# xbarin02/libdwt

Hardware: AMD Instinct MI355X
Metric: Gsamples/s (= % HBM3E BW) CDF 9/7 2-D fwd float, 8192^2 5-level (higher is better)
Workload: dtype f32

## Files before the change

### libdwt_amd/csrc/dwt_abi.hip

```cpp
#include "dwt_backend.h"

#include <climits>

using namespace dwtb;

namespace {
enum OptKind { kPlain, kSweep , kBool, kNonNegative };
struct Opt {
	const char *name;
	int *(*ref)(Ctx &);
	OptKind kind;
};
#define DWT_OPT(name_, member_, kind_) {name_, [](Ctx &c) -> int * { return &c.member_; }, kind_}
const Opt kOpts[] = {
	DWT_OPT("generic", force_generic, kSweep), DWT_OPT("eaw_two_pass", eaw_two_pass, kBool), DWT_OPT("feat_groups", feat_groups, kNonNegative), DWT_OPT("swt_fused", swt_fused, kBool), DWT_OPT("cond_fused", cond_fused, kPlain), DWT_OPT("timefreq_tiled", tf_tiled, kBool), DWT_OPT("cpt", tune.cpt, kSweep), DWT_OPT("tile_pairs", tune.tile_pairs, kSweep),
	DWT_OPT("waves", tune.waves, kSweep), DWT_OPT("xcd_swizzle", tune.xcd_swizzle, kSweep), DWT_OPT("ring", tune.ring, kSweep),
	DWT_OPT("ring_inv", tune.ring_inv, kSweep), DWT_OPT("inv_ll_temporal", tune.inv_ll_temporal, kSweep), DWT_OPT("inv_pairs", tune.inv_pairs, kSweep), DWT_OPT("nt", tune.nt, kSweep), DWT_OPT("nt_auto", tune.nt_auto, kSweep),
	DWT_OPT("fma", fma, kSweep), DWT_OPT("fused_d", fused_d, kPlain), DWT_OPT("ride_copy", ride_copy, kBool), DWT_OPT("ride_mib", ride_mib, kNonNegative), DWT_OPT("il_exact_borders", il_exact_borders, kPlain),
	DWT_OPT("il_inplace_shell", il_inplace_shell, kPlain), DWT_OPT("host_pipeline", host_pipeline, kPlain),
	DWT_OPT("tune_tiles", tune_tiles, kPlain), DWT_OPT("tune_in_call", tune_in_call, kBool), DWT_OPT("place_tries", place_tries, kPlain),
	DWT_OPT("place_min_mib", place_min_mib, kNonNegative), DWT_OPT("place_max_gib", place_max_gib, kNonNegative),
	DWT_OPT("vol_ip_waves", vol.ip_waves, kPlain), DWT_OPT("vol_tile_pairs", vol.tile_pairs, kPlain), DWT_OPT("vol_nt", vol.nt, kPlain),
	DWT_OPT("vol_fused", vol.fused, kPlain), DWT_OPT("vol_direct", vol.direct, kPlain), DWT_OPT("vol_whole", vol.whole, kPlain),
	DWT_OPT("vol_inplace_fused", vol.inplace_fused, kBool), DWT_OPT("vol_swizzle", vol.swizzle, kPlain), DWT_OPT("vol_rows", vol.rows, kPlain),
};
#undef DWT_OPT
const Opt *find_opt(const char *name)
{
	for (const Opt &o : kOpts)
		if (!strcmp(name, o.name))
			return &o;
	return nullptr;
}
}

#pragma GCC visibility push(default)
extern "C" {

const char *dwt_hip_last_error(void) { return g_err; }

int dwt_hip_device_count(void)
{
	int n = 0;
	if (hipGetDeviceCount(&n) != hipSuccess)
		return 0;
	return n;
}

int dwt_hip_init(void)
{
	if (g.inited)
// ... 445 lines not shown
```

### libdwt_amd/csrc/dwt_backend.h

```cpp
#pragma once
#include "../../include/libdwt_hip.h"
#include "dwt_kernels.h"

#include <hip/hip_runtime.h>
#include <stdarg.h>
#include <stdio.h>
#include <stdlib.h>
#include <string.h>
#include <algorithm>
#include <array>
#include <condition_variable>
#include <functional>
#include <initializer_list>
#include <map>
#include <mutex>
#include <thread>
#include <unistd.h>
#include <utility>
#include <vector>

namespace dwtb {
using namespace dwt;

struct Buf {
// ... 23 lines not shown
		return std::array{&stage_img, &ll[0], &ll[1], &frame_a, &frame_b, &vol_out, &vol_host[0], &vol_host[1], &eaw_w, &eaw_ll[0], &eaw_ll[1], &feat_ws, &swt_ws, &cond_ws, &band_ws};
	}
	hipEvent_t dl_ev[8] = {};
	hipEvent_t switch_ev = nullptr;
	hipStream_t up = nullptr, down = nullptr;
	hipEvent_t pipe_ev[3][16] = {};
	int host_pipeline = 1;
	void *pin = nullptr;
	size_t pin_bytes = 0;
	int feat_groups = 0;
	int tf_tiled = 1;
	int cond_fused = -1;
	int swt_fused = 1;
	SweepTuning tune;
	VolTuning vol;
	int force_generic = 0;
	int eaw_two_pass = 0;
	int fma = 0;
	int il_temporal = 0;
	int il_inplace_shell = 1;
	int il_exact_borders = 1;
	int tune_tiles = 1;
	std::map<unsigned long long, int> tile_cache;
	int place_tries = 4;
	int place_min_mib = 1024;
	int place_max_gib = 0;
	int tune_in_call = -1;
	bool tuning = false;
	bool placing = false;
	long stat_launches = 0, stat_allocs = 0;
	double place_ms[8] = {0};
	int place_n = 0, place_best = -1;
	int fused_d = 1;
	int ride_copy = 1;
	int ride_mib = 32;
	int prof_on = 0;
	std::vector<std::pair<hipEvent_t, hipEvent_t>> prof_events;
	std::vector<int> prof_tag;
	size_t prof_used = 0;
	double prof_ms = 0;
	int prof_launches = 0;
	double prof_level_ms[16] = {0};
	int prof_level_n[16] = {0};
};

extern thread_local Ctx g;
extern thread_local char g_err[512];
extern thread_local bool g_elems_are_32bit;

int fail(const char *fmt, ...);
int launched(hipError_t e, const char *family, const char *what);
int check_dev_align(std::initializer_list<const void *> ptrs, std::initializer_list<long> strides);
inline bool overlap(const void *a, size_t na, const void *b, size_t nb)
{
	const uintptr_t pa = (uintptr_t)a, pb = (uintptr_t)b;
	return na && nb && pa < pb + nb && pb < pa + na;
}

static inline bool wavelet_of(int id, Wavelet *w)
{
	if (id >= 0 && id <= 5) {
		*w = (Wavelet)id;
		return true;
	}
	if (id == DWT_HIP_INTERP53_S) {
		*w = kInterp53S;
// ... 34 lines not shown
	bool dense() const { return sox == six && soy == siy; }
};

int grow(Buf &b, size_t need);
void dev_free(void *p);
void drop(Buf &b);
int grant_range(const void *p, int owner, const int *devices, int n_devices);
int copy_rect_on(hipStream_t st, Img dst, long dx, long dy, Img src, long sx_, long sy_, long w, long h);
int copy_rect(Img dst, long dx, long dy, Img src, long sx_, long sy_, long w, long h);
int zero_rect(Img img, long x, long y, long w, long h);
struct Frame {
	void *p;
	long sx, sy;
	int es, w, h;
	bool dev;
};
int frame_check(const Frame &f);
int frame_pack(const Frame &f, void *dense, long pitch);
int frame_unpack(const Frame &f, const void *dense, long pitch);
inline long frame_pitch(long es, long w) { return align_up(es * w, 256); }
int frame_stage(const Frame &f, Buf &buf, Img *dense);
int frame_pack_stack(Frame f, int n, long plane_stride, void *stack, long pitch);
int frame_unpack_stack(Frame f, int n, long plane_stride, const void *stack, long pitch);
int host_volume_xfer(bool to_device, void *dev, size_t d_sy, size_t d_sz, void *host, size_t h_sy, size_t h_sz, int nx, int ny, int nz);
int generic_pass(Wavelet w, bool inverse, bool rows, Img in, Img out, int frame_w, int frame_h, int n_lines, int N, int hoff);
size_t ll_band_bytes(const Geom &ge, int k, int batch, int es);
int timed_forward(Wavelet w, Img s, Img d, const Geom &ge, int levels, int batch, long sb, long db, double *ms);
int place_ll_scratch(Wavelet w, Img s, Img d, const Geom &ge, int levels, int batch, long sb, long db);
int tune2d(Wavelet w, bool inverse, Img s, Img d, const Geom &ge, int levels, int batch, long sb, long db);
bool stream_is_capturing();
bool may_measure();
int tuned_tile_pairs(Wavelet w, const FwdLevelArgs &a);
int tuned_tile_pairs(Wavelet w, const InvLevelArgs &a);
void apply_tile_choice(int choice, SweepTuning *t, bool inverse);
int forward2d(Wavelet w, Img src, Img dst, const Geom &ge, int *jp, int decompose_one, int zero_padding, int batch, long src_bstride, long dst_bstride);
int inverse2d(Wavelet w, Img src, Img dst, const Geom &ge, int j_max, int decompose_one, int zero_padding, int batch, long src_bstride, long dst_bstride);
bool level_fused_ok(const Geom &ge, int j);
int transform1d(Wavelet w, bool inverse, const void *src, void *dst, long line_stride, long elem_stride, int n_lines,
	int so, int si, int *jp, int zero_padding);
int host_forward_pipelined(Wavelet w, const void *src, void *dst, int stride_x, int W, int H, int *jp, int decompose_one);
int host_inverse_pipelined(Wavelet w, const void *src, void *dst, int stride_x, int W, int H, int j_max, int decompose_one);
bool swt_fused_ok(const void *src, long ls, long es, int N);
int swt_device(Wavelet w, const char *src, long ls, long es, int n_lines, int N, int level0, int levels, char *dst_h, long h_es,
	char *dst_l, long l_es, int l_mode, long plane_stride, long dls);
int band_abs_median(const void *ptr, long bstride, int batch, long stride_x, int fw, int fh, int x0, int y0, int w, int h, float *med);
int prof_drain();
void prof_before(int level = 0);
void prof_after(int level = 0);
int check_inited();

}
```

### libdwt_amd/csrc/dwt_backend.hip

```cpp
#include "dwt_backend.h"

namespace dwtb {

thread_local Ctx g;
thread_local char g_err[512] = "";

int fail(const char *fmt, ...)
{
	va_list ap;
	va_start(ap, fmt);
	vsnprintf(g_err, sizeof(g_err), fmt, ap);
	va_end(ap);
	return 1;
}

int launched(hipError_t e, const char *family, const char *what)
{
	g.stat_launches++;
	return e == hipSuccess ? 0 : fail("%s %s launch failed: %s", family, what, hipGetErrorString(e));
}

int check_dev_align(std::initializer_list<const void *> ptrs, std::initializer_list<long> strides)
{
	bool ok = true;
// ... 171 lines not shown
	g.prof_used = 0;
	return 0;
}

long ll_pitch_elems(int w) { return align_up(w, 4); }
static char *ll_band(int k) { return (char *)g.ll[k].p; }

size_t ll_band_bytes(const Geom &ge, int k, int batch, int es)
{
	return (size_t)ll_pitch_elems(ge.Wo(k + 1)) * ge.Ho(k + 1) * es * batch + 64;
}

int ensure_ll(const Geom &ge, int batch, int es)
{
	for (int k = 0; k < 2; k++) {
		if (g.ll_external) {
			if (g.ll[k].bytes < ll_band_bytes(ge, k, batch, es))
				return fail("the caller's workspace (dwt_hip_set_workspace) is too small: band %d needs %zu bytes", k, ll_band_bytes(ge, k, batch, es));
			continue;
		}
		if (grow(g.ll[k], ll_band_bytes(ge, k, batch, es)))
			return 1;
	}
	return 0;
}

thread_local bool g_elems_are_32bit = true;

bool level_fused_ok(const Geom &ge, int j)
{
	return !g.force_generic && (g_elems_are_32bit || g.fused_d) && ge.Wi(j) == ge.Wo(j) && ge.Hi(j) == ge.Ho(j) && ge.Wo(j) >= 2 &&
		ge.Ho(j) >= 2;
}
int forward2d(Wavelet w, Img src, Img dst, const Geom &ge, int *jp, int decompose_one, int zero_padding,
	int batch, long src_bstride, long dst_bstride)
{
	const int so_min = ge.sox < ge.soy ? ge.sox : ge.soy, so_max = ge.sox > ge.soy ? ge.sox : ge.soy;
	const int j_limit = ceil_log2(decompose_one ? so_max : so_min);
	if (*jp < 0 || *jp > j_limit)
		*jp = j_limit;
	const int J = *jp;
	if (J == 0)
		return 0;
	const int es = elem_size(w);
	const bool dbl = es == 8;
	if (ensure_ll(ge, batch, es))
		return 1;

	int ll_in = -1;
	Img cur = src;
	RideCopy ride;
	auto carriers_from = [&](int j0) {
		int n = 0;
		for (int j = j0; j < J && level_fused_ok(ge, j); j++)
			n += !dbl && sweep_ride_ok(g.tune, ge.Wo(j), ge.Ho(j), batch, false);
		return n;
	};
	for (int j = 0; j < J; j++) {
		const int Wo = ge.Wo(j), Ho = ge.Ho(j), Wi = ge.Wi(j), Hi = ge.Hi(j);
		const int Wd = ge.Wo(j + 1), Hd = ge.Ho(j + 1);
		if (level_fused_ok(ge, j)) {
			const bool last = (j == J - 1) || !level_fused_ok(ge, j + 1);
			FwdLevelArgs a;
			a.W = Wo;
			a.H = Ho;
			a.batch = batch;
			bool detour = false;
			if (ll_in < 0) {
				a.in = cur.p;
				a.in_pitch = cur.sx / es;
				a.in_bstride = (cur.p == src.p ? src_bstride : dst_bstride) / es;
				detour = (cur.p == dst.p);
			} else {
				a.in = ll_band(ll_in);
				a.in_pitch = ll_pitch_elems(Wo);
				a.in_bstride = a.in_pitch * Ho;
			}
			Img hdst = dst;
			long h_bstride = dst_bstride;
			if (detour) {
				if (batch != 1)
					return fail("in-place batches are not supported; use distinct src and dst");
				if (grow(g.stage_img, (size_t)dst.sx * Ho))
					return 1;
				hdst = Img{(char *)g.stage_img.p, dst.sx, es};
				h_bstride = 0;
				a.temporal = (g.ride_copy && carriers_from(j + 1) > 0) ? 0 : 1;
			}
			a.out_h = hdst.p;
			a.h_pitch = hdst.sx / es;
			a.h_bstride = h_bstride / es;
			const int ll_out = last ? -1 : (ll_in < 0 ? (j & 1) : 1 - ll_in);
			if (last) {
				a.out_ll = hdst.p;
				a.ll_pitch = a.h_pitch;
				a.ll_bstride = a.h_bstride;
			} else {
				a.out_ll = ll_band(ll_out);
				a.ll_pitch = ll_pitch_elems(Wd);
				a.ll_bstride = a.ll_pitch * Hd;
			}
			SweepTuning tune = g.tune;
			if (!dbl && tune.tile_pairs <= 0)
				apply_tile_choice(tuned_tile_pairs(w, a), &tune, false);
			if (ride.on && ride.next < ride.total && !dbl && sweep_ride_ok(tune, Wo, Ho, batch, false)) {
				a.ride = &ride.r;
				a.ride_lo = ride.next;
				a.ride_hi = ride.next + ride.share((size_t)Wo * Ho * es, carriers_from(j + 1));
				ride.next = a.ride_hi;
			}
			prof_before(j);
			hipError_t e = dbl ? launch_fwd_level_d(w, a, tune, g.stream)
			                   : launch_fwd_level((g.fma && w == kCdf97S) ? kCdf97SFma : w, a, tune, g.stream);
			prof_after(j);
			if (e != hipSuccess)
				return fail("forward level %d launch failed: %s", j, hipGetErrorString(e));
			if (detour) {
				const Rect rc[3] = {{Wd, 0, Wd, 0, Wo - Wd, Ho}, {0, Hd, 0, Hd, Wd, Ho - Hd}, {0, 0, 0, 0, last ? Wd : 0, Hd}};
				ride.r = make_copy_rects(dst, hdst, rc, 3, 3);
				ride.total = copy_rects_plan(&ride.r);
				ride.next = 0;
				ride.on = g.ride_copy && ride.total > 0 && carriers_from(j + 1) > 0;
				if (!ride.on && copy_rects_on(g.stream, dst, hdst, rc, 3))
					return 1;
			}
			ll_in = ll_out;
			cur = dst;
			continue;
		}

		if (ride.flush())
			return 1;
		if (batch != 1)
			return fail("batched transforms need dense frames with both sides >= 2 at every level");
		if (ll_in >= 0) {
			Img s{ll_band(ll_in), ll_pitch_elems(Wo) * es, es};
			if (copy_rect(dst, 0, 0, s, 0, 0, Wo, Ho))
				return 1;
			ll_in = -1;
			cur = dst;
		}
		if (Wi == Wo && Hi == Ho && Wo >= 2 && Ho >= 2) {
			if (grow(g.stage_img, (size_t)dst.sx * Ho))
				return 1;
			const Img S{(char *)g.stage_img.p, dst.sx, dst.es};
			if (generic_pass(w, false, true, cur, S, Wo, Ho, Ho, Wi, Wd) || generic_pass(w, false, false, S, dst, Wo, Ho, Wo, Hi, Hd))
				return 1;
			cur = dst;
		} else {
			if (!skip_single(w) || Wo > 1) {
				if (generic_pass(w, false, true, cur, dst, Wo, Ho, Ho, Wi, Wd))
					return 1;
				cur = dst;
			}
			if (!skip_single(w) || Ho > 1) {
				if (generic_pass(w, false, false, cur, dst, Wo, Ho, Wo, Hi, Hd))
					return 1;
				cur = dst;
			}
		}
// ... 181 lines not shown
```

### libdwt_amd/csrc/dwt_kernels.h

```cpp
#pragma once
#include <hip/hip_runtime.h>
#include <stddef.h>

namespace dwt {

enum Wavelet { kCdf97S = 0, kCdf53I = 1, kCdf53S = 2, kCdf97D = 3, kCdf53D = 4, kCdf97I = 5,
	kCdf97SFma = 6 ,
	kCdf53SNew = 7 ,
	kCdf97IIp = 8 ,
	kInterp53S = 9  };

inline int elem_size(Wavelet w) { return (w == kCdf97D || w == kCdf53D) ? 8 : 4; }

struct SweepTuning {
	int cpt = 0;
	int tile_pairs = 0;
	int waves = 4;
	int xcd_swizzle = 1;
	int ring = 0;
	int nt = 7;
	int nt_auto = 1;
	int ring_inv = 8;
	int inv_pairs = 0;
	int inv_ll_temporal = 1;
// ... 31 lines not shown
	int il_ll = 0;
	int temporal = 0;
	int pair_lo = 0, pair_hi = 0;
	IlShell sh;
	const CopyRects *ride = nullptr;
	int ride_lo = 0, ride_hi = 0;
	int unused = 0;
	int out_step = 1;
};

struct InvLevelArgs {
	const void *in_ll;
	long ll_pitch, ll_bstride;
	const void *in_h;
	long h_pitch, h_bstride;
	void *out;
	long out_pitch, out_bstride;
	int W, H, batch;
	int interleaved = 0;
	int plain_ends = 0;
	int temporal_out = 0;
	int pair_lo = 0, pair_hi = 0;
	const CopyRects *ride = nullptr;
	int ride_lo = 0, ride_hi = 0;
	IlShell sh;
	int in_step = 1;
	const void *in_ll2 = nullptr;
	long ll2_pitch = 0;
};

struct IlStripArgs;
hipError_t launch_fwd_level(Wavelet w, const FwdLevelArgs &a, const SweepTuning &t, hipStream_t s, const IlStripArgs *strip = nullptr);

hipError_t launch_inv_level(Wavelet w, const InvLevelArgs &a, const SweepTuning &t, hipStream_t s, const IlStripArgs *strip = nullptr);
hipError_t launch_fwd_level_d(Wavelet w, const FwdLevelArgs &a, const SweepTuning &t, hipStream_t s);
hipError_t launch_inv_level_d(Wavelet w, const InvLevelArgs &a, const SweepTuning &t, hipStream_t s);
bool have_fused_inverse(Wavelet w);

hipError_t launch_line_pass(Wavelet w, bool inverse, const void *src, void *dst, long line_stride, long elem_stride,
	int n_lines, int N, int hoff, bool lanes_along_lines, hipStream_t s);

constexpr int N1D_MAX = 8192;
hipError_t launch_line_levels(Wavelet w, bool inverse, const void *src, void *dst, long line_stride, long elem_stride,
	int n_lines, int N, int levels, hipStream_t s);

hipError_t launch_eaw_line(bool inverse, const void *src, long ls, long es, int n_lines, int N, int hoff, float *tmp, float *w,
	bool lanes_along_lines, float alpha, hipStream_t s);
hipError_t launch_eaw_place(void *dst, long ls, long es, int n_lines, int N, int hoff, const float *tmp, bool lanes_along_lines, hipStream_t s);
struct EawLevelArgs {
	const float *in = nullptr;
	float *ll_out = nullptr, *det_out = nullptr, *wH_out = nullptr, *wV_out = nullptr;
	const float *ll = nullptr, *det = nullptr, *wH = nullptr, *wV = nullptr;
	float *out = nullptr;
	long pin = 0, pll = 0, pd = 0, pout = 0;
	long bi_in = 0, bi_ll = 0, bi_det = 0, bi_w = 0, bi_out = 0;
	int W = 0, H = 0, batch = 1;
};
hipError_t launch_eaw_level(bool inverse, const EawLevelArgs &a, float alpha, hipStream_t s);
hipError_t launch_eaw97_line(bool inverse, const void *src, long ls, long es, int n_lines, int N, int hoff, float *tmp, float *w,
	bool lanes_along_lines, float alpha, hipStream_t s);
hipError_t launch_eaw97_level(bool inverse, const EawLevelArgs &a, float alpha, hipStream_t s);

struct VolTuning {
	int cpt = 8;
	int tile_pairs = 0;
	int nt = -1;
// ... 241 lines not shown
```

### libdwt_amd/csrc/dwt_sweep2d.hip

```cpp
#include "dwt_sweep2d.h"

namespace dwt {

template <class W, bool INV>
__global__ __launch_bounds__(256) void k_line_pass(const char *__restrict__ src, char *__restrict__ dst,
	long line_stride, long elem_stride, int n_lines, int N, int hoff, int lanes_along_lines)
{
	using T = typename W::T;
	constexpr int K = W::K;
	const int fast = blockIdx.x * blockDim.x + threadIdx.x;
	const int slow = blockIdx.y;
	const int line = lanes_along_lines ? fast : slow;
	const int k = lanes_along_lines ? slow : fast;
	const int npairs = (N + 1) >> 1;
	if (line >= n_lines || k >= npairs)
		return;
	const char *s = src + (long)line * line_stride;
	char *d = dst + (long)line * line_stride;
	auto ld = [&](int idx) { return *(const T *)(s + (long)idx * elem_stride); };
	auto st = [&](int idx, T v) { *(T *)(d + (long)idx * elem_stride) = v; };
	const bool il = hoff < 0;

	if (N == 1) {
		if (W::kScaleSingle)
// ... 75 lines not shown
		if (v & 2)
			continue;
		constexpr int P = 2;
		const f2 ov = f2{row[0][v], row[0][v + P]}, ev = f2{row[1][v], row[1][v + P]};
		f2 s_[K], n_[K], lo2, hi2;
#pragma unroll
		for (int i = 0; i < K; i++)
			s_[i] = f2{st[i][v], st[i][v + P]};
		n_[0] = ev;
		n_[1] = ov + kk(0) * (tap(0, s_[0]) + ev);
		if constexpr (K == 4) {
			n_[2] = s_[0] + kk(1) * (tap(1, s_[1]) + n_[1]);
			n_[3] = s_[1] + kk(2) * (tap(2, s_[2]) + n_[2]);
			const f2 s2n = s_[2] + kk(3) * (tap(3, s_[3]) + n_[3]);
			lo2 = s2n * zl;
			hi2 = n_[3] * zh;
		} else {
			const f2 s1n = s_[0] + kk(1) * (tap(1, s_[1]) + n_[1]);
			lo2 = s1n * zl;
			hi2 = n_[1] * zh;
		}
#pragma unroll
		for (int i = 0; i < K; i++) {
			st[i][v] = n_[i][0];
			st[i][v + P] = n_[i][1];
		}
		lo[v] = lo2[0];
		lo[v + P] = lo2[1];
		hi[v] = hi2[0];
		hi[v + P] = hi2[1];
	}
}

template <class W, int CPT, int RING, int NT, bool IL, bool X>
static __device__ __forceinline__ void fwd_sweep_tile(const FwdLevelArgs &a, const SweepGeom &g)
{
	using T = typename W::T;
	constexpr int K = W::K;
	constexpr int kRing = RING;
	constexpr int kAhead = kRing / 2 - 1;
	constexpr int kLdAux = (NT & 2) ? 2 : 0;
	constexpr bool kNtStore = (NT & 1) != 0;
	[[maybe_unused]] constexpr bool kNtStoreLL = kNtStore && !(NT & 4);
	constexpr bool kShuffle = (NT & 8) != 0;
	constexpr int TW = 64 * CPT;
	constexpr int RS = TW + 8;
	constexpr int HK = (K + 1) & ~1;
	constexpr int NARR = CPT + 2 * HK;
	constexpr int kDmaPerIter = 2 * (CPT / 4 + 1);
	constexpr bool kPairRows = kIsSelEnds<W> && std::is_same<T, float>::value && has_coef_ends<W>::value && !std::is_base_of<Cdf97SFma, W>::value;
	extern __shared__ __attribute__((aligned(16))) char smem[];

	const int lane = threadIdx.x & 63, nwv = blockDim.x >> 6;
	const int wv = __builtin_amdgcn_readfirstlane(threadIdx.x >> 6);
	const int bid = tile_block_id(g.swz, X ? g.first : 0, g.tile_blocks);
	int tx, ty;
	if (g.wave_horiz) {
		const int ntxb = (g.ntx + nwv - 1) / nwv;
		tx = (bid % ntxb) * nwv + wv;
		ty = bid / ntxb;
	} else {
		tx = bid % g.ntx;
		ty = (bid / g.ntx) * nwv + wv;
	}
	const int img = blockIdx.y;
	const int Wd = (a.W + 1) >> 1, Hd = (a.H + 1) >> 1;
	const int A = ty * g.tile_pairs;
	if (A >= Hd || tx >= g.ntx)
		return;
	if (a.pair_hi > 0 && (A < a.pair_lo || A >= a.pair_hi))
		return;
	const int B = min(A + g.tile_pairs, Hd);
	const int c0 = tx * TW;
	const int n_iter = (B - A) + K;
	const int q0 = A - K / 2;

	const T *in = (const T *)a.in + (long)img * a.in_bstride;
	T *out_ll = (T *)a.out_ll + (long)img * a.ll_bstride;
	T *out_h = (T *)a.out_h + (long)img * a.h_bstride;

	char *ring = smem + (size_t)wv * kRing * RS * 4;
	const unsigned ring_off = lds_offset(ring);

	const int n_edge = min(4, c0 + TW - a.W);
	const int edge_col = kIsSelEnds<W> ? a.W - 2 - min(lane, 3) : reflect(a.W + min(lane, 3), a.W);
	const int halo_i = lane < 4 ? c0 - 4 + lane : c0 + TW + (lane & 3);
	const int halo_col = kIsSelEnds<W> ? reflect_near(halo_i, a.W) : reflect(halo_i, a.W);

	int islot = 0, rslot = 0;
	const bool tall = kIsSelEnds<W> || a.H >= 64;
	[[maybe_unused]] const bool shl = IL && a.sh.rows != nullptr;
	[[maybe_unused]] int halo_sh = -1;
	if (IL && shl)
		halo_sh = (halo_col >= c0 - 4 && halo_col < c0) ? 8 * (tx - 1) + (halo_col - (c0 - 4))
			: (halo_col >= c0 + TW && halo_col < c0 + TW + 4) ? 8 * tx + 4 + (halo_col - (c0 + TW)) : -1;
	auto issue = [&](int it) {
#pragma unroll
		for (int rr = 0; rr < 2; rr++) {
			const int ri = 2 * (q0 + it) - 1 + rr;
			const int r = tall ? reflect1(ri, a.H) : reflect(ri, a.H);
			char *lrow = ring + (size_t)(islot + rr) * RS * 4;
			const T *grow = in + (long)r * a.in_pitch;
			[[maybe_unused]] const T *hsrc = grow + halo_col;
			[[maybe_unused]] const T *rgt = nullptr;
			if (IL && shl) {
				if (r < 2 * A)
					grow = (const T *)a.sh.rows + (long)(9 * (ty - 1) + r - (2 * A - 5)) * a.sh.rows_pitch, hsrc = grow + halo_col;
				else if (r >= 2 * B)
					grow = (const T *)a.sh.rows + (long)(9 * ty + r - (2 * B - 5)) * a.sh.rows_pitch, hsrc = grow + halo_col;
				else if (r < kIlKeepTop)
					grow = (const T *)a.sh.top + (long)r * a.sh.top_pitch, hsrc = grow + halo_col;
				else {
					rgt = (const T *)a.sh.right + (long)r * a.sh.right_pitch - a.sh.right_x0;
					if (halo_sh >= 0)
						hsrc = (const T *)a.sh.cols + (long)r * a.sh.cols_pitch + halo_sh;
					else if (halo_col >= a.W - kIlKeepRight)
						hsrc = rgt + halo_col;
				}
			}
			[[maybe_unused]] const T *esrc = (IL && rgt) ? rgt + edge_col : grow + edge_col;
			const bool fix_right = IL && rgt && c0 + TW > a.W - kIlKeepRight;
			const row_rsrc_t rs = row_rsrc(grow, (unsigned)a.W * 4);
			if (kLdAux != 0 && it < K && A > 0) {
#pragma unroll
				for (int i = 0; i < CPT / 4; i++)
					dma16_row<0>(rs, (unsigned)(c0 + i * 256 + lane * 4) * 4, lrow + i * 1024);
				if (fix_right && lane < kIlKeepRight)
					dma4<0>(rgt + (a.W - kIlKeepRight + lane), lrow + (a.W - kIlKeepRight - c0) * 4);
				if (lane < n_edge)
					dma4<0>(esrc, lrow + (a.W - c0) * 4);
				if (lane < 8)
					dma4<0>(IL ? hsrc : grow + halo_col, lrow + TW * 4);
			} else {
#pragma unroll
				for (int i = 0; i < CPT / 4; i++)
					dma16_row<kLdAux>(rs, (unsigned)(c0 + i * 256 + lane * 4) * 4, lrow + i * 1024);
				if (fix_right && lane < kIlKeepRight)
					dma4<0>(rgt + (a.W - kIlKeepRight + lane), lrow + (a.W - kIlKeepRight - c0) * 4);
				if (lane < n_edge)
					dma4<kLdAux>(esrc, lrow + (a.W - c0) * 4);
				if (lane < 8)
					dma4<0>(IL ? hsrc : grow + halo_col, lrow + TW * 4);
			}
		}
		islot = islot + 2 >= kRing ? 0 : islot + 2;
	};

	T st[K][CPT];
#pragma unroll
	for (int s = 0; s < K; s++)
#pragma unroll
		for (int v = 0; v < CPT; v++)
			st[s][v] = 0;

	[[maybe_unused]] unsigned hends = 0;
	[[maybe_unused]] bool h_any = false, h_simple = false;
	constexpr unsigned kCand = (1u << HK) | (1u << (HK + CPT - 1));
	if constexpr (W::kEndForms) {
		hends = end_mask<NARR>(c0 + lane * CPT - HK, a.W);
		h_any = !a.plain_ends && __builtin_amdgcn_ballot_w64(hends != 0) != 0;
		h_simple = __builtin_amdgcn_ballot_w64((hends & ~(kCand | 1u | (1u << (NARR - 1)))) != 0) == 0;
	}
	[[maybe_unused]] bool e0 = false, e1 = false;
	[[maybe_unused]] T kh[K];
	if constexpr (kIsSelEnds<W>) {
		const unsigned m = end_mask_long<NARR>(c0 + lane * CPT - HK, a.W);
		e0 = (m >> HK) & 1;
		e1 = (m >> (HK + CPT - 1)) & 1;
		sel_coefs<W, false, HK>(kh, e0, e1);
	}
	[[maybe_unused]] auto row_is_end = [&](int r) {
		if (tall || kIsSelEnds<W>)
			return r == 0 || r == a.H - 1;
		const int rr = reflect(r, a.H);
		return rr == 0 || rr == a.H - 1;
	};

	for (int it = 0; it < kAhead && it < n_iter; it++)
		issue(it);

	for (int it = 0; it < n_iter; it++) {
		if (it + kAhead < n_iter) {
			issue(it + kAhead);
			DWT_WAIT_VMCNT(kAhead * kDmaPerIter);
		} else {
			DWT_WAIT_VMCNT(0);
		}

		T row[2][CPT];
		[[maybe_unused]] T xs[2][kPairRows ? NARR : 1];
#pragma unroll
		for (int rr = 0; rr < 2; rr++) {
			const unsigned base = ring_off + (unsigned)(rslot + rr) * RS * 4;
			const unsigned own = base + lane * CPT * 4;
			const unsigned la = lane == 0 ? base + TW * 4 : own - 16;
			const unsigned ra = lane == 63 ? base + TW * 4 + 16 : own + CPT * 4;
			T x[NARR];
			u4 L4, R4, O0, O1;
			if constexpr (kShuffle) {
				u4 H4;
				const unsigned ha = base + TW * 4 + (lane == 63 ? 16 : 0);
				if constexpr (CPT == 8) {
// ... 40 lines not shown
				if (__builtin_expect(!h_any, 1)) {
					lift_fwd_regs<W, NARR>(x, 0u);
				} else if (h_simple) {
					DWT_END_PATH();
					lift_fwd_regs<W, NARR, kCand>(x, hends);
				} else {
					DWT_END_PATH();
					lift_fwd_regs<W, NARR>(x, hends);
				}
			} else if constexpr (kIsSelEnds<W>) {
				lift_regs_sel<W, NARR, false, HK, HK + CPT - 1>(x, e0, e1, kh);
			} else {
				lift_fwd_regs<W, NARR>(x, 0u);
			}
#pragma unroll
			for (int v = 0; v < CPT; v++)
				row[rr][v] = W::fwd_scale(v & 1, x[HK + v]);
		}

		if constexpr (kPairRows) {
			typedef float f2 __attribute__((ext_vector_type(2)));
			f2 x2[NARR];
#pragma unroll
			for (int j = 0; j < NARR; j++)
				x2[j] = f2{xs[0][j], xs[1][j]};
#pragma unroll
			for (int s_ = 0; s_ < K; s_++) {
#pragma unroll
				for (int j = s_ + 1; j <= NARR - 2 - s_; j += 2) {
					if (j == HK)
						x2[j] = x2[j] + kh[s_] * ((e0 ? f2{-0.0f, -0.0f} : x2[j - 1]) + x2[j + 1]);
					else if (j == HK + CPT - 1)
						x2[j] = x2[j] + kh[s_] * (x2[j - 1] + (e1 ? f2{-0.0f, -0.0f} : x2[j + 1]));
					else
						x2[j] = x2[j] + W::fk(s_) * (x2[j - 1] + x2[j + 1]);
				}
			}
			const float ze = W::fwd_scale(0, 1.0f), zo = W::fwd_scale(1, 1.0f);
#pragma unroll
			for (int v = 0; v < CPT; v++) {
				const f2 sc = x2[HK + v] * ((v & 1) ? zo : ze);
				row[0][v] = sc[0];
				row[1][v] = sc[1];
			}
		}
		rslot = rslot + 2 >= kRing ? 0 : rslot + 2;

		[[maybe_unused]] bool vend[K] = {};
		[[maybe_unused]] bool v_any = false;
		if constexpr (W::kEndForms) {
#pragma unroll
			for (int s_ = 0; s_ < K; s_++) {
				vend[s_] = row_is_end(2 * (q0 + it) - 1 - s_);
				v_any = !a.plain_ends && (v_any || vend[s_]);
			}
		}
		T lo[CPT], hi[CPT];
		auto vertical = [&](auto ends_tag) {
			constexpr bool ENDS = decltype(ends_tag)::value;
			if constexpr (kPairRows && !ENDS && K != 1) {
				vertical_pairs<W, CPT>(row, st, lo, hi);
				return;
			}
#pragma unroll
			for (int v = 0; v < CPT; v++) {
				const T ov = row[0][v], ev = row[1][v];
// ... 109 lines not shown
#pragma unroll
					for (int e = 0; e < CPT; e += 4)
						store8_row<false>(dl, (unsigned)(c0 + lane * CPT) * 2 + e * 2, u2{to_bits(lo[e]), to_bits(lo[e + 2])});
				}
			} else
			if (it >= K && (!X || A + it - K >= kIlKeepTop / 2)) {
				const int k = A + it - K;
				const unsigned cb = (unsigned)(c0 + lane * CPT) * 4;
				const T *r0 = out_h + (long)(2 * k) * a.h_pitch;
				const unsigned row_bytes = (unsigned)(X ? a.W - kIlKeepRight : a.W) * 4;
				const row_rsrc_t d0 = row_rsrc(r0, row_bytes);
#pragma unroll
				for (int e = 0; e < CPT; e += 4) {
					const u4 v4{to_bits(lo[e]), to_bits(lo[e + 1]), to_bits(lo[e + 2]), to_bits(lo[e + 3])};
					if (a.il_ll == 2)
						store16_row<false>(d0, cb + e * 4, v4);
					else
						store16_row<kNtStore>(d0, cb + e * 4, v4);
				}
				if (2 * k + 1 < a.H) {
					const row_rsrc_t d1 = row_rsrc(r0 + a.h_pitch, row_bytes);
#pragma unroll
					for (int e = 0; e < CPT; e += 4)
						store16_row<kNtStore>(d1, cb + e * 4, u4{to_bits(hi[e]), to_bits(hi[e + 1]), to_bits(hi[e + 2]), to_bits(hi[e + 3])});
				}
				if (a.il_ll) {
					const row_rsrc_t dl = row_rsrc(out_ll + (long)k * a.ll_pitch, (unsigned)(X ? (a.W - kIlKeepRight + 1) >> 1 : Wd) * 4);
#pragma unroll
					for (int e = 0; e < CPT; e += 4)
						store8_row<false>(dl, cb / 2 + e * 2, u2{to_bits(lo[e]), to_bits(lo[e + 2])});
				}
			}
		} else
		if (it >= K) {
			const int k = A + it - K;
			const unsigned clb = (unsigned)((c0 + lane * CPT) >> 1) * 4;
			const T *top = out_h + (long)k * a.h_pitch, *bot = out_h + (long)(Hd + k) * a.h_pitch;
			const unsigned nlb = (unsigned)Wd * 4, nhb = (unsigned)(a.W >> 1) * 4;
			const row_rsrc_t dll = row_rsrc(out_ll + (long)k * a.ll_pitch, nlb), dhl = row_rsrc(top + Wd, nhb);
			const bool hrow = k < (a.H >> 1);
			if constexpr (CPT == 8) {
				store16_row<kNtStoreLL>(dll, clb, u4{to_bits(lo[0]), to_bits(lo[2]), to_bits(lo[4]), to_bits(lo[6])});
				store16_row<kNtStore>(dhl, clb, u4{to_bits(lo[1]), to_bits(lo[3]), to_bits(lo[5]), to_bits(lo[7])});
				if (hrow) {
					store16_row<kNtStore>(row_rsrc(bot, nlb), clb, u4{to_bits(hi[0]), to_bits(hi[2]), to_bits(hi[4]), to_bits(hi[6])});
					store16_row<kNtStore>(row_rsrc(bot + Wd, nhb), clb, u4{to_bits(hi[1]), to_bits(hi[3]), to_bits(hi[5]), to_bits(hi[7])});
				}
			} else {
				store8_row<kNtStoreLL>(dll, clb, u2{to_bits(lo[0]), to_bits(lo[2])});
				store8_row<kNtStore>(dhl, clb, u2{to_bits(lo[1]), to_bits(lo[3])});
				if (hrow) {
					store8_row<kNtStore>(row_rsrc(bot, nlb), clb, u2{to_bits(hi[0]), to_bits(hi[2])});
					store8_row<kNtStore>(row_rsrc(bot + Wd, nhb), clb, u2{to_bits(hi[1]), to_bits(hi[3])});
				}
			}
		}
	}
}

template <class W, int CPT, int RING, int NT, bool IL, bool X>
static __device__ __forceinline__ void fwd_sweep_any_tile(const FwdLevelArgs &a, const SweepGeom &g)
{
	if constexpr (W::kEndForms) {
		if (a.plain_ends)
			fwd_sweep_tile<PlainEnds<W>, CPT, RING, NT, IL, X>(a, g);
		else if (a.W % CPT == 0 && a.W >= 64 && a.H >= 64)
			fwd_sweep_tile<SelEnds<W>, CPT, RING, NT, IL, X>(a, g);
		else
			fwd_sweep_tile<W, CPT, RING, NT, IL, X>(a, g);
	} else
		fwd_sweep_tile<W, CPT, RING, NT, IL, X>(a, g);
}

template <class W, int CPT, int RING, int NT, bool IL = false>
__global__ __launch_bounds__(256) void k_fwd_sweep(FwdLevelArgs a, SweepGeom g)
{
	fwd_sweep_any_tile<W, CPT, RING, NT, IL, false>(a, g);
}

template <class W, int CPT, int RING, int NT>
__global__ __launch_bounds__(256) void k_fwd_sweep_r(FwdLevelArgs a, SweepGeom g, CopyRects r)
{
	if ((int)blockIdx.x >= g.tile_blocks) {
		ride_copy_block(r, (int)blockIdx.x - g.tile_blocks);
		return;
	}
	fwd_sweep_any_tile<W, CPT, RING, NT, false, false>(a, g);
}

template <class W, int CPT, int RING, int NT>
__global__ __launch_bounds__(256) void k_fwd_sweep_x(FwdLevelArgs a, SweepGeom g, IlStripArgs strip)
{
	if ((int)blockIdx.x < g.first) {
		il_strip_wave<W, false>(strip, blockIdx.x * (blockDim.x >> 6) + (threadIdx.x >> 6));
		return;
	}
	fwd_sweep_any_tile<W, CPT, RING, NT, true, true>(a, g);
}

template <class W, int CPT, int RING, int NT, bool IL = false>
static hipError_t fwd_launch(const FwdLevelArgs &a, const SweepGeom &g, dim3 grid, int waves, hipStream_t s)
{
	const size_t lds = (size_t)waves * RING * (64 * CPT + 8) * 4;
	if constexpr (!IL && RING == 8 && (NT == 7 || NT == 3)) {
		if (a.ride && a.ride_hi > a.ride_lo) {
			if (hipError_t e = allow_lds((const void *)k_fwd_sweep_r<W, CPT, RING, NT>, lds))
				return e;
			SweepGeom gr = g;
			gr.tile_blocks = (int)grid.x;
			CopyRects r = *a.ride;
// ... 65 lines not shown
	if (g.wave_horiz)
		grid = dim3(((g.ntx + waves - 1) / waves) * nty, a.batch);
	else
		grid = dim3(g.ntx * ((nty + waves - 1) / waves), a.batch);
	if (a.sh.rows && (!a.interleaved || a.batch != 1 || a.out_step != 1 || g.tile_pairs != a.sh.tile_pairs))
		return hipErrorInvalidValue;
	if (a.ride && a.ride_hi > a.ride_lo && (a.interleaved || a.batch != 1 || waves != 4 || tt.ring != 8 || a.temporal || (tt.nt & 8)))
		return hipErrorInvalidValue;
	if (a.interleaved) {
		if constexpr (std::is_same<W, Cdf97S>::value || std::is_same<W, Cdf53SNew>::value) {
			if (strip) {
				if (a.batch != 1 || a.W < 64 || a.H < 64)
					return hipErrorInvalidValue;
				return tt.ring == 16 ? fwd_launch_x<W, 16>(a, g, grid, waves, *strip, s) : fwd_launch_x<W, 8>(a, g, grid, waves, *strip, s);
			}
		}
		if (strip)
			return hipErrorInvalidValue;
		if constexpr (std::is_base_of<Cdf97S, W>::value || std::is_base_of<Cdf53S, W>::value) {
			if (tt.ring == 16)
				return fwd_launch<W, 4, 16, 3, true>(a, g, grid, waves, s);
			return fwd_launch<W, 4, 8, 3, true>(a, g, grid, waves, s);
		} else {
			return hipErrorInvalidValue;
		}
	}
	if (strip)
		return hipErrorInvalidValue;
	if (tt.nt_auto && (tt.nt & 12) == 4 && (size_t)a.batch * ((a.W + 1) / 2) * ((a.H + 1) / 2) * sizeof(typename W::T) >= ((size_t)1 << 30))
		tt.nt = 3;
	return cpt == 8 ? fwd_pick<W, 8>(a, g, grid, waves, tt, s) : fwd_pick<W, 4>(a, g, grid, waves, tt, s);
}

bool sweep_ride_ok(const SweepTuning &t, int W, int H, int batch, bool inverse)
{
	if (batch != 1 || W < 2 || H < 2 || !(t.waves >= 1 && t.waves <= 4 ? t.waves == 4 : true) || (t.nt & 8))
		return false;
	if (inverse)
		return t.ring_inv != 16;
	if (t.ring == 16)
		return false;
	if (t.ring == 8)
		return true;
	const int cpt = pick_cpt(t, W, false);
	const int tp = pick_tile_pairs(t, W, H, cpt, 1);
	const long ntx = (W + 64 * cpt - 1) / (64 * cpt), nty = ((H + 1) / 2 + tp - 1) / tp;
	return !(ntx >= 4 && ntx * nty >= 3072);
}

int il_sweep_tile_pairs(const SweepTuning &t, int W, int H, bool inverse)
{
	return pick_tile_pairs(t, W, H, 4, 1, inverse, true);
}

hipError_t launch_fwd_level(Wavelet w, const FwdLevelArgs &a, const SweepTuning &t, hipStream_t s, const IlStripArgs *strip)
{
	if (strip && w != kCdf97S && w != kCdf53SNew)
		return hipErrorInvalidValue;
	switch (w) {
	case kCdf97S: return fwd_level_t<Cdf97S>(a, t, s, strip);
	case kCdf53I: return fwd_level_t<Cdf53I>(a, t, s);
	case kCdf53S: return fwd_level_t<Cdf53S>(a, t, s);
	case kCdf97I: return fwd_level_t<Cdf97I>(a, t, s);
	case kCdf97SFma: return fwd_level_t<Cdf97SFma>(a, t, s);
	case kCdf53SNew: return a.interleaved ? fwd_level_t<Cdf53SNew>(a, t, s, strip) : hipErrorInvalidValue;
	case kInterp53S: return a.interleaved ? hipErrorInvalidValue : fwd_level_t<Interp53S>(a, t, s);
// ... 7 lines not shown
```

### libdwt_amd/csrc/dwt_tuning.hip

```cpp
#include "dwt_backend.h"

namespace dwtb {

bool may_measure()
{
	if (g.tune_in_call < 0) {
		const char *e = getenv("DWT_HIP_TUNE");
		g.tune_in_call = (e && atoi(e) > 0) ? 1 : 0;
	}
	return g.tuning || g.tune_in_call > 0;
}

struct TileCand {
	int pairs, cpt, ring;
};
static int pack_choice(const TileCand &c) { return c.pairs | (c.cpt << 16) | (c.ring << 24); }

void apply_tile_choice(int choice, SweepTuning *t, bool inverse)
{
	if (choice <= 0)
		return;
	t->tile_pairs = choice & 0xffff;
	if ((choice >> 16) & 0xff)
		t->cpt = (choice >> 16) & 0xff;
// ... 42 lines not shown
			fprintf(stderr, "tune %s W %d: %d pairs, cpt %d, ring %d: %.1f us%s\n", inverse ? "inv" : "fwd", (int)((key >> 38) & 0xfffff), c.pairs, c.cpt, c.ring,
				ms * 1e3, ok ? "" : " (failed)");
		if (ok && (!best || ms < best_ms)) {
			best = pack_choice(c);
			best_ms = ms;
		}
	}
	hipEventDestroy(e0);
	hipEventDestroy(e1);
	(void)hipGetLastError();
	g.tile_cache[key] = best;
	return best;
}

static unsigned long long tile_key(Wavelet w, bool inverse, int W, int H, int batch)
{
	return ((unsigned long long)w << 59) ^ ((unsigned long long)inverse << 58) ^ ((unsigned long long)W << 38) ^ ((unsigned long long)H << 18) ^ (unsigned long long)batch;
}

static bool tunable(int W, int H, int batch, int interleaved)
{
	return g.tune_tiles && !interleaved && (size_t)W * H * batch * sizeof(float) >= ((size_t)512 << 20) && W >= 1024 && H >= 256;
}

int tuned_tile_pairs(Wavelet w, const FwdLevelArgs &a)
{
	if (!tunable(a.W, a.H, a.batch, a.interleaved))
		return 0;
	const Wavelet wk = (g.fma && w == kCdf97S) ? kCdf97SFma : w;
	return tune_tile_pairs(tile_key(w, false, a.W, a.H, a.batch), false, {{64, 0, 0}, {32, 0, 0}, {16, 0, 0}},
		[&](const SweepTuning &t) { return launch_fwd_level(wk, a, t, g.stream); });
}

int tuned_tile_pairs(Wavelet w, const InvLevelArgs &a)
{
	if (!tunable(a.W, a.H, a.batch, a.interleaved))
		return 0;
	const Wavelet wk = (g.fma && w == kCdf97S) ? kCdf97SFma : w;
	return tune_tile_pairs(tile_key(w, true, a.W, a.H, a.batch), true, {{16, 0, 0}, {32, 0, 0}, {8, 0, 0}, {16, 8, 0}, {32, 8, 0}},
		[&](const SweepTuning &t) { return launch_inv_level(wk, a, t, g.stream); });
}
int timed_forward(Wavelet w, Img s, Img d, const Geom &ge, int levels, int batch, long sb, long db, double *ms)
{
	hipEvent_t e0, e1;
	HIP_TRY(hipEventCreate(&e0));
	HIP_TRY(hipEventCreate(&e1));
	int rc = 0;
	g.placing = true;
	for (int r = 0; r < 2 && !rc; r++) {
		int j = levels;
		hipEventRecord(e0, g.stream);
		rc = forward2d(w, s, d, ge, &j, 0, 0, batch, sb, db);
		hipEventRecord(e1, g.stream);
	}
	g.placing = false;
	float t = 0;
	if (!rc && (hipEventSynchronize(e1) != hipSuccess || hipEventElapsedTime(&t, e0, e1) != hipSuccess))
		rc = fail("timing a placement trial failed: %s", hipGetErrorString(hipGetLastError()));
	hipEventDestroy(e0);
	hipEventDestroy(e1);
	*ms = t;
	return rc;
}

static size_t place_jump(int k)
{
// ... 140 lines not shown
```

Before: 575.8.

## Fuse first two forward CDF 9/7 levels into one sweep kernel

Adds a fused kernel that computes level 0 of the float CDF 9/7 forward transform and feeds its LL rows straight into a level-1 lifting pass held in registers. Level 1's horizontal lift uses cross-lane shuffles and its vertical lift a register ring, writing both levels' detail bands and the level-1 LL. This avoids the HBM write and re-read of the level-0 LL band and one kernel launch, at the cost of overlapping tiles with halo recomputation, warm-up rows and higher register pressure. A heuristic gate and a separate tile-size tuning entry decide when the fused pair is used.

```diff
diff --git a/libdwt_amd/csrc/dwt_abi.hip b/libdwt_amd/csrc/dwt_abi.hip
--- a/libdwt_amd/csrc/dwt_abi.hip
+++ b/libdwt_amd/csrc/dwt_abi.hip
@@ -16,7 +16,7 @@
 	DWT_OPT("generic", force_generic, kSweep), DWT_OPT("eaw_two_pass", eaw_two_pass, kBool), DWT_OPT("feat_groups", feat_groups, kNonNegative), DWT_OPT("swt_fused", swt_fused, kBool), DWT_OPT("cond_fused", cond_fused, kPlain), DWT_OPT("timefreq_tiled", tf_tiled, kBool), DWT_OPT("cpt", tune.cpt, kSweep), DWT_OPT("tile_pairs", tune.tile_pairs, kSweep),
 	DWT_OPT("waves", tune.waves, kSweep), DWT_OPT("xcd_swizzle", tune.xcd_swizzle, kSweep), DWT_OPT("ring", tune.ring, kSweep),
 	DWT_OPT("ring_inv", tune.ring_inv, kSweep), DWT_OPT("inv_ll_temporal", tune.inv_ll_temporal, kSweep), DWT_OPT("inv_pairs", tune.inv_pairs, kSweep), DWT_OPT("nt", tune.nt, kSweep), DWT_OPT("nt_auto", tune.nt_auto, kSweep),
-	DWT_OPT("fma", fma, kSweep), DWT_OPT("fused_d", fused_d, kPlain), DWT_OPT("ride_copy", ride_copy, kBool), DWT_OPT("ride_mib", ride_mib, kNonNegative), DWT_OPT("il_exact_borders", il_exact_borders, kPlain),
+	DWT_OPT("fma", fma, kSweep), DWT_OPT("fused_d", fused_d, kPlain), DWT_OPT("fuse01", fuse01, kPlain), DWT_OPT("ride_copy", ride_copy, kBool), DWT_OPT("ride_mib", ride_mib, kNonNegative), DWT_OPT("il_exact_borders", il_exact_borders, kPlain),
 	DWT_OPT("il_inplace_shell", il_inplace_shell, kPlain), DWT_OPT("host_pipeline", host_pipeline, kPlain),
 	DWT_OPT("tune_tiles", tune_tiles, kPlain), DWT_OPT("tune_in_call", tune_in_call, kBool), DWT_OPT("place_tries", place_tries, kPlain),
 	DWT_OPT("place_min_mib", place_min_mib, kNonNegative), DWT_OPT("place_max_gib", place_max_gib, kNonNegative),
diff --git a/libdwt_amd/csrc/dwt_backend.h b/libdwt_amd/csrc/dwt_backend.h
--- a/libdwt_amd/csrc/dwt_backend.h
+++ b/libdwt_amd/csrc/dwt_backend.h
@@ -79,6 +79,7 @@
 	double place_ms[8] = {0};
 	int place_n = 0, place_best = -1;
 	int fused_d = 1;
+	int fuse01 = 1;
 	int ride_copy = 1;
 	int ride_mib = 32;
 	int prof_on = 0;
@@ -179,6 +180,7 @@
 bool may_measure();
 int tuned_tile_pairs(Wavelet w, const FwdLevelArgs &a);
 int tuned_tile_pairs(Wavelet w, const InvLevelArgs &a);
+int tuned_tile_pairs01(Wavelet w, const FwdLevelArgs &a);
 void apply_tile_choice(int choice, SweepTuning *t, bool inverse);
 int forward2d(Wavelet w, Img src, Img dst, const Geom &ge, int *jp, int decompose_one, int zero_padding, int batch, long src_bstride, long dst_bstride);
 int inverse2d(Wavelet w, Img src, Img dst, const Geom &ge, int j_max, int decompose_one, int zero_padding, int batch, long src_bstride, long dst_bstride);
diff --git a/libdwt_amd/csrc/dwt_backend.hip b/libdwt_amd/csrc/dwt_backend.hip
--- a/libdwt_amd/csrc/dwt_backend.hip
+++ b/libdwt_amd/csrc/dwt_backend.hip
@@ -227,6 +227,20 @@
 	return !g.force_generic && (g_elems_are_32bit || g.fused_d) && ge.Wi(j) == ge.Wo(j) && ge.Hi(j) == ge.Ho(j) && ge.Wo(j) >= 2 &&
 		ge.Ho(j) >= 2;
 }
+static bool pair01_ok(Wavelet w, const Geom &ge, int J, int batch)
+{
+	const int W = ge.Wo(0), H = ge.Ho(0);
+	if (!g.fuse01 || g.fma || J < 2 || !level_fused_ok(ge, 0) || !level_fused_ok(ge, 1) || !fwd01_can(w, W, H))
+		return false;
+	const SweepTuning &t = g.tune;
+	if (t.cpt == 4 || t.ring == 8 || (t.nt & 8) || (t.tile_pairs & 1))
+		return false;
+	if (g.fuse01 >= 2)
+		return true;
+	const long ntx = (W + 511) / 512, nty = ((H >> 1) + 63) / 64;
+	return fwd01_tiles(W) * 10 <= ntx * 11 && ntx * nty * batch >= 32768;
+}
+
 int forward2d(Wavelet w, Img src, Img dst, const Geom &ge, int *jp, int decompose_one, int zero_padding,
 	int batch, long src_bstride, long dst_bstride)
 {
@@ -255,7 +269,9 @@
 		const int Wo = ge.Wo(j), Ho = ge.Ho(j), Wi = ge.Wi(j), Hi = ge.Hi(j);
 		const int Wd = ge.Wo(j + 1), Hd = ge.Ho(j + 1);
 		if (level_fused_ok(ge, j)) {
-			const bool last = (j == J - 1) || !level_fused_ok(ge, j + 1);
+			const bool pair = j == 0 && ll_in < 0 && cur.p != dst.p && pair01_ok(w, ge, J, batch);
+			const int jl = pair ? j + 1 : j;
+			const bool last = (jl == J - 1) || !level_fused_ok(ge, jl + 1);
 			FwdLevelArgs a;
 			a.W = Wo;
 			a.H = Ho;
@@ -285,19 +301,19 @@
 			a.out_h = hdst.p;
 			a.h_pitch = hdst.sx / es;
 			a.h_bstride = h_bstride / es;
-			const int ll_out = last ? -1 : (ll_in < 0 ? (j & 1) : 1 - ll_in);
+			const int ll_out = last ? -1 : (ll_in < 0 ? (jl & 1) : 1 - ll_in);
 			if (last) {
 				a.out_ll = hdst.p;
 				a.ll_pitch = a.h_pitch;
 				a.ll_bstride = a.h_bstride;
 			} else {
 				a.out_ll = ll_band(ll_out);
-				a.ll_pitch = ll_pitch_elems(Wd);
-				a.ll_bstride = a.ll_pitch * Hd;
+				a.ll_pitch = ll_pitch_elems(ge.Wo(jl + 1));
+				a.ll_bstride = a.ll_pitch * ge.Ho(jl + 1);
 			}
 			SweepTuning tune = g.tune;
 			if (!dbl && tune.tile_pairs <= 0)
-				apply_tile_choice(tuned_tile_pairs(w, a), &tune, false);
+				apply_tile_choice(pair ? tuned_tile_pairs01(w, a) : tuned_tile_pairs(w, a), &tune, false);
 			if (ride.on && ride.next < ride.total && !dbl && sweep_ride_ok(tune, Wo, Ho, batch, false)) {
 				a.ride = &ride.r;
 				a.ride_lo = ride.next;
@@ -305,8 +321,9 @@
 				ride.next = a.ride_hi;
 			}
 			prof_before(j);
-			hipError_t e = dbl ? launch_fwd_level_d(w, a, tune, g.stream)
-			                   : launch_fwd_level((g.fma && w == kCdf97S) ? kCdf97SFma : w, a, tune, g.stream);
+			hipError_t e = pair ? launch_fwd01(a, tune, g.stream)
+			             : dbl  ? launch_fwd_level_d(w, a, tune, g.stream)
+			                    : launch_fwd_level((g.fma && w == kCdf97S) ? kCdf97SFma : w, a, tune, g.stream);
 			prof_after(j);
 			if (e != hipSuccess)
 				return fail("forward level %d launch failed: %s", j, hipGetErrorString(e));
@@ -321,6 +338,7 @@
 			}
 			ll_in = ll_out;
 			cur = dst;
+			j = jl;
 			continue;
 		}
 
diff --git a/libdwt_amd/csrc/dwt_kernels.h b/libdwt_amd/csrc/dwt_kernels.h
--- a/libdwt_amd/csrc/dwt_kernels.h
+++ b/libdwt_amd/csrc/dwt_kernels.h
@@ -87,6 +87,10 @@
 struct IlStripArgs;
 hipError_t launch_fwd_level(Wavelet w, const FwdLevelArgs &a, const SweepTuning &t, hipStream_t s, const IlStripArgs *strip = nullptr);
 
+bool fwd01_can(Wavelet w, int W, int H);
+int fwd01_tiles(int W);
+hipError_t launch_fwd01(const FwdLevelArgs &a, const SweepTuning &t, hipStream_t s);
+
 hipError_t launch_inv_level(Wavelet w, const InvLevelArgs &a, const SweepTuning &t, hipStream_t s, const IlStripArgs *strip = nullptr);
 hipError_t launch_fwd_level_d(Wavelet w, const FwdLevelArgs &a, const SweepTuning &t, hipStream_t s);
 hipError_t launch_inv_level_d(Wavelet w, const InvLevelArgs &a, const SweepTuning &t, hipStream_t s);
diff --git a/libdwt_amd/csrc/dwt_sweep2d.hip b/libdwt_amd/csrc/dwt_sweep2d.hip
--- a/libdwt_amd/csrc/dwt_sweep2d.hip
+++ b/libdwt_amd/csrc/dwt_sweep2d.hip
@@ -131,9 +131,10 @@
 	}
 }
 
-template <class W, int CPT, int RING, int NT, bool IL, bool X>
+template <class W, int CPT, int RING, int NT, bool IL, bool X, bool F01 = false>
 static __device__ __forceinline__ void fwd_sweep_tile(const FwdLevelArgs &a, const SweepGeom &g)
 {
+	static_assert(!F01 || (kIsSelEnds<W> && CPT == 8 && !IL && !X && W::K == 4 && !(NT & 8)), "the fused pair: float 9/7 by selection, Mallat");
 	using T = typename W::T;
 	constexpr int K = W::K;
 	constexpr int kRing = RING;
@@ -154,6 +155,11 @@
 	const int wv = __builtin_amdgcn_readfirstlane(threadIdx.x >> 6);
 	const int bid = tile_block_id(g.swz, X ? g.first : 0, g.tile_blocks);
 	int tx, ty;
+	if constexpr (F01) {
+		const int t = bid * nwv + wv;
+		tx = t % g.ntx;
+		ty = t / g.ntx;
+	} else
 	if (g.wave_horiz) {
 		const int ntxb = (g.ntx + nwv - 1) / nwv;
 		tx = (bid % ntxb) * nwv + wv;
@@ -170,9 +176,10 @@
 	if (a.pair_hi > 0 && (A < a.pair_lo || A >= a.pair_hi))
 		return;
 	const int B = min(A + g.tile_pairs, Hd);
-	const int c0 = tx * TW;
-	const int n_iter = (B - A) + K;
-	const int q0 = A - K / 2;
+	const int c0 = tx * (F01 ? TW - 32 : TW);
+	const int warm = (F01 && A > 0) ? K : 0;
+	const int n_iter = (B - A) + K + warm + (F01 ? 3 : 0);
+	const int q0 = A - K / 2 - warm;
 
 	const T *in = (const T *)a.in + (long)img * a.in_bstride;
 	T *out_ll = (T *)a.out_ll + (long)img * a.ll_bstride;
@@ -220,7 +227,7 @@
 			[[maybe_unused]] const T *esrc = (IL && rgt) ? rgt + edge_col : grow + edge_col;
 			const bool fix_right = IL && rgt && c0 + TW > a.W - kIlKeepRight;
 			const row_rsrc_t rs = row_rsrc(grow, (unsigned)a.W * 4);
-			if (kLdAux != 0 && it < K && A > 0) {
+			if (kLdAux != 0 && it < K + warm && A > 0) {
 #pragma unroll
 				for (int i = 0; i < CPT / 4; i++)
 					dma16_row<0>(rs, (unsigned)(c0 + i * 256 + lane * 4) * 4, lrow + i * 1024);
@@ -267,6 +274,19 @@
 		e0 = (m >> HK) & 1;
 		e1 = (m >> (HK + CPT - 1)) & 1;
 		sel_coefs<W, false, HK>(kh, e0, e1);
+	}
+	[[maybe_unused]] bool e1m = false, g0 = false, g5 = false, g7 = false, g9 = false, own0 = true, own1 = true;
+	[[maybe_unused]] T st1[K][4] = {}, held[4] = {};
+	if constexpr (F01) {
+		e1m = c0 + lane * CPT + 3 == a.W - 1;
+		const unsigned m1 = end_mask_long<12>((c0 >> 1) + lane * 4 - 4, a.W >> 1);
+		g0 = (m1 >> 4) & 1;
+		g5 = (m1 >> 5) & 1;
+		g7 = (m1 >> 7) & 1;
+		g9 = (m1 >> 9) & 1;
+		const bool last_tile = tx == g.ntx - 1;
+		own0 = last_tile || lane < 60;
+		own1 = (tx == 0 || lane >= 1) && (last_tile || lane <= 60);
 	}
 	[[maybe_unused]] auto row_is_end = [&](int r) {
 		if (tall || kIsSelEnds<W>)
@@ -373,6 +393,8 @@
 						x2[j] = x2[j] + kh[s_] * ((e0 ? f2{-0.0f, -0.0f} : x2[j - 1]) + x2[j + 1]);
 					else if (j == HK + CPT - 1)
 						x2[j] = x2[j] + kh[s_] * (x2[j - 1] + (e1 ? f2{-0.0f, -0.0f} : x2[j + 1]));
+					else if (F01 && j == HK + 3)
+						x2[j] = x2[j] + (e1m ? 2.0f * W::fk(s_) : W::fk(s_)) * (x2[j - 1] + (e1m ? f2{-0.0f, -0.0f} : x2[j + 1]));
 					else
 						x2[j] = x2[j] + W::fk(s_) * (x2[j - 1] + x2[j + 1]);
 				}
@@ -548,6 +570,91 @@
 				}
 			}
 		} else
+		if constexpr (F01) {
+			typedef float f2 __attribute__((ext_vector_type(2)));
+			const f2 nz = f2{-0.0f, -0.0f};
+			const int k = q0 + it - K / 2;
+			if (k >= A && k < B && own0) {
+				const unsigned clb = (unsigned)((c0 + lane * CPT) >> 1) * 4;
+				const T *top = out_h + (long)k * a.h_pitch, *bot = out_h + (long)(Hd + k) * a.h_pitch;
+				const unsigned nb = (unsigned)Wd * 4;
+				store16_row<kNtStore>(row_rsrc(top + Wd, nb), clb, u4{to_bits(lo[1]), to_bits(lo[3]), to_bits(lo[5]), to_bits(lo[7])});
+				store16_row<kNtStore>(row_rsrc(bot, nb), clb, u4{to_bits(hi[0]), to_bits(hi[2]), to_bits(hi[4]), to_bits(hi[6])});
+				store16_row<kNtStore>(row_rsrc(bot + Wd, nb), clb, u4{to_bits(hi[1]), to_bits(hi[3]), to_bits(hi[5]), to_bits(hi[7])});
+			}
+			if (it & 1) {
+#pragma unroll
+				for (int e = 0; e < 4; e++)
+					held[e] = lo[2 * e];
+			} else {
+				const int q1 = k >> 1, W1 = Wd, H1 = Hd;
+				f2 y[12];
+#pragma unroll
+				for (int e = 0; e < 4; e++) {
+					const unsigned b0 = to_bits(held[e]), b1 = to_bits(lo[2 * e]);
+					y[e] = f2{from_bits<T>(from_left_lane(b0)), from_bits<T>(from_left_lane(b1))};
+					y[4 + e] = f2{held[e], lo[2 * e]};
+					y[8 + e] = f2{from_bits<T>(from_right_lane(b0)), from_bits<T>(from_right_lane(b1))};
+				}
+#pragma unroll
+				for (int s_ = 0; s_ < K; s_++) {
+#pragma unroll
+					for (int j = s_ + 1; j <= 10 - s_; j += 2) {
+						if (j == 4 || j == 5 || j == 7 || j == 9) {
+							const bool el = j == 4 && g0, er = j == 5 ? g5 : j == 7 ? g7 : j == 9 ? g9 : false;
+							y[j] = y[j] + ((el || er) ? 2.0f * W::fk(s_) : W::fk(s_)) * ((el ? nz : y[j - 1]) + (er ? nz : y[j + 1]));
+						} else
+							y[j] = y[j] + W::fk(s_) * (y[j - 1] + y[j + 1]);
+					}
+				}
+				const float ze = W::fwd_scale(0, 1.0f), zo = W::fwd_scale(1, 1.0f);
+				bool vt[K], vb[K];
+				T kv[K];
+#pragma unroll
+				for (int s_ = 0; s_ < K; s_++) {
+					vt[s_] = 2 * q1 - 1 - s_ == 0;
+					vb[s_] = 2 * q1 - 1 - s_ == H1 - 1;
+					kv[s_] = (vt[s_] || vb[s_]) ? 2.0f * W::fk(s_) : W::fk(s_);
+				}
+				auto older = [&](int s_, f2 v) { return vt[s_] ? nz : v; };
+				auto newer = [&](int s_, f2 v) { return vb[s_] ? nz : v; };
+				T lo1[4], hi1[4];
+#pragma unroll
+				for (int v = 0; v < 2; v++) {
+					const f2 c0v = y[4 + v] * (v ? zo : ze), c2v = y[6 + v] * (v ? zo : ze);
+					const f2 ov = f2{c0v[0], c2v[0]}, ev = f2{c0v[1], c2v[1]};
+					f2 s_[K], n_[K];
+#pragma unroll
+					for (int i = 0; i < K; i++)
+						s_[i] = f2{st1[i][v], st1[i][v + 2]};
+					n_[0] = ev;
+					n_[1] = ov + kv[0] * (older(0, s_[0]) + newer(0, ev));
+					n_[2] = s_[0] + kv[1] * (older(1, s_[1]) + newer(1, n_[1]));
+					n_[3] = s_[1] + kv[2] * (older(2, s_[2]) + newer(2, n_[2]));
+					const f2 s2n = s_[2] + kv[3] * (older(3, s_[3]) + newer(3, n_[3]));
+					const f2 l2 = s2n * ze, h2 = n_[3] * zo;
+#pragma unroll
+					for (int i = 0; i < K; i++) {
+						st1[i][v] = n_[i][0];
+						st1[i][v + 2] = n_[i][1];
+					}
+					lo1[v] = l2[0];
+					lo1[v + 2] = l2[1];
+					hi1[v] = h2[0];
+					hi1[v + 2] = h2[1];
+				}
+				const int k1 = q1 - K / 2;
+				if (k1 >= (A >> 1) && k1 < (B >> 1) && own1) {
+					const int W2 = W1 >> 1, H2 = H1 >> 1;
+					const unsigned cb = (unsigned)((c0 >> 2) + lane * 2) * 4, nb = (unsigned)W2 * 4;
+					const T *top = out_h + (long)k1 * a.h_pitch, *bot = out_h + (long)(H2 + k1) * a.h_pitch;
+					store8_row<kNtStoreLL>(row_rsrc(out_ll + (long)k1 * a.ll_pitch, nb), cb, u2{to_bits(lo1[0]), to_bits(lo1[2])});
+					store8_row<kNtStore>(row_rsrc(top + W2, nb), cb, u2{to_bits(lo1[1]), to_bits(lo1[3])});
+					store8_row<kNtStore>(row_rsrc(bot, nb), cb, u2{to_bits(hi1[0]), to_bits(hi1[2])});
+					store8_row<kNtStore>(row_rsrc(bot + W2, nb), cb, u2{to_bits(hi1[1]), to_bits(hi1[3])});
+				}
+			}
+		} else
 		if (it >= K) {
 			const int k = A + it - K;
 			const unsigned clb = (unsigned)((c0 + lane * CPT) >> 1) * 4;
@@ -592,6 +699,12 @@
 __global__ __launch_bounds__(256) void k_fwd_sweep(FwdLevelArgs a, SweepGeom g)
 {
 	fwd_sweep_any_tile<W, CPT, RING, NT, IL, false>(a, g);
+}
+
+template <int NT>
+__global__ __launch_bounds__(256) void k_fwd_sweep01(FwdLevelArgs a, SweepGeom g)
+{
+	fwd_sweep_tile<SelEnds<Cdf97S>, 8, 16, NT, false, false, true>(a, g);
 }
 
 template <class W, int CPT, int RING, int NT>
@@ -723,6 +836,49 @@
 	return cpt == 8 ? fwd_pick<W, 8>(a, g, grid, waves, tt, s) : fwd_pick<W, 4>(a, g, grid, waves, tt, s);
 }
 
+bool fwd01_can(Wavelet w, int W, int H)
+{
+	return Cdf97S::kEndForms && w == kCdf97S && W % 4 == 0 && H % 4 == 0 && W >= 128 && H >= 128;
+}
+
+int fwd01_tiles(int W)
+{
+	const int W1 = W >> 1;
+	return W1 <= 256 ? 1 : (W1 - 256 + 239) / 240 + 1;
+}
+
+hipError_t launch_fwd01(const FwdLevelArgs &a, const SweepTuning &t, hipStream_t s)
+{
+	if (!fwd01_can(kCdf97S, a.W, a.H) || a.batch < 1 || a.interleaved || a.ride || a.pair_hi > 0 || (t.tile_pairs & 1))
+		return hipErrorInvalidValue;
+	const int waves = t.waves >= 1 && t.waves <= 4 ? t.waves : 4;
+	const int Hd = a.H >> 1;
+	SweepGeom g;
+	g.ntx = fwd01_tiles(a.W);
+	g.swz = t.xcd_swizzle;
+	g.wave_horiz = 1;
+	g.tile_pairs = t.tile_pairs;
+	if (g.tile_pairs <= 0) {
+		g.tile_pairs = 64;
+		while (g.tile_pairs > 16 && (long)g.ntx * ((Hd + g.tile_pairs - 1) / g.tile_pairs) * a.batch < 1024)
+			g.tile_pairs >>= 1;
+	}
+	const long tiles = (long)g.ntx * ((Hd + g.tile_pairs - 1) / g.tile_pairs);
+	const dim3 grid((unsigned)((tiles + waves - 1) / waves), a.batch);
+	const size_t lds = (size_t)waves * 16 * (64 * 8 + 8) * 4;
+	const bool ll_nt = !(t.nt & 4) || (t.nt_auto && (size_t)a.batch * (a.W >> 2) * (a.H >> 2) * sizeof(float) >= ((size_t)1 << 30));
+	if (ll_nt) {
+		if (hipError_t e = allow_lds((const void *)k_fwd_sweep01<3>, lds))
+			return e;
+		k_fwd_sweep01<3><<<grid, 64 * waves, lds, s>>>(a, g);
+	} else {
+		if (hipError_t e = allow_lds((const void *)k_fwd_sweep01<7>, lds))
+			return e;
+		k_fwd_sweep01<7><<<grid, 64 * waves, lds, s>>>(a, g);
+	}
+	return hipGetLastError();
+}
+
 bool sweep_ride_ok(const SweepTuning &t, int W, int H, int batch, bool inverse)
 {
 	if (batch != 1 || W < 2 || H < 2 || !(t.waves >= 1 && t.waves <= 4 ? t.waves == 4 : true) || (t.nt & 8))
diff --git a/libdwt_amd/csrc/dwt_tuning.hip b/libdwt_amd/csrc/dwt_tuning.hip
--- a/libdwt_amd/csrc/dwt_tuning.hip
+++ b/libdwt_amd/csrc/dwt_tuning.hip
@@ -98,6 +98,14 @@
 		[&](const SweepTuning &t) { return launch_fwd_level(wk, a, t, g.stream); });
 }
 
+int tuned_tile_pairs01(Wavelet w, const FwdLevelArgs &a)
+{
+	if (!tunable(a.W, a.H, a.batch, a.interleaved))
+		return 0;
+	return tune_tile_pairs(tile_key(w, false, a.W, a.H, a.batch) ^ (1ull << 63), false, {{64, 0, 0}, {128, 0, 0}, {32, 0, 0}},
+		[&](const SweepTuning &t) { return launch_fwd01(a, t, g.stream); });
+}
+
 int tuned_tile_pairs(Wavelet w, const InvLevelArgs &a)
 {
 	if (!tunable(a.W, a.H, a.batch, a.interleaved))
```

New measurement: 601.8, median of 6. 1.05x the previous value.
